# ucb-bar/Accelerated-TinyMPC

Measured on AMD Instinct MI355X. Metric: MPC solves/sec (batched quadrotor nx=12,nu=4,N=30), higher is better.
Workload: dtype f32; 1 GPU; quadrotor_tracking batched 65536 instances per GPU, cold-start tiny_solve, early_exit (tol 1e-3, max_iter 100); nx=12, nu=4, N=30, instances_per_gpu=65536, instances_total=65536, parallelism=batch-shard x1, world_size_seen=1, backend=none (single process), kernel=tile16<12,4,30,exact>, max_iters=85

## Files before the change

### accelerated-tinympc_amd/csrc/admm_tile16.hip

```cpp
#include "rowlane_math.h"
#include <cstdlib>

namespace tinympc
{

typedef float f32x16 __attribute__((ext_vector_type(16)));
#ifndef TINY_T16_ABLATE
#define TINY_T16_ABLATE 0
#endif
#ifndef TINY_T16_CQ
#define TINY_T16_CQ 1
#endif
#ifndef TINY_T16_BADDR
#define TINY_T16_BADDR 1
#endif
#ifndef TINY_T16_PADTAB
#define TINY_T16_PADTAB 1
#endif
#ifndef TINY_T16_XPOSE
#define TINY_T16_XPOSE 1
#endif
#ifndef TINY_T16_SCHED
#define TINY_T16_SCHED 1
#endif
#ifndef TINY_T16_LINES
#define TINY_T16_LINES 1
#endif
#ifndef TINY_T16_STAMP
#define TINY_T16_STAMP 0
#endif

#if TINY_T16_ABLATE == 1
__device__ __forceinline__ f32x4 t16_fake4(float a, float b, f32x4 c) { c[0] += a; c[1] += b; c[2] += a; c[3] += b; return c; }
#define TINY_MFMA4(a, b, c) t16_fake4((a), (b), (c))
#define TINY_MFMA1(a, b, c) __builtin_amdgcn_mfma_f32_16x16x1f32((a), (b), (c), 0, 0, 0)
#else
#define TINY_MFMA4(a, b, c) __builtin_amdgcn_mfma_f32_16x16x4f32((a), (b), (c), 0, 0, 0)
#define TINY_MFMA1(a, b, c) __builtin_amdgcn_mfma_f32_16x16x1f32((a), (b), (c), 0, 0, 0)
#endif

template <int V>
__device__ __forceinline__ void gather12(float (&t)[12], const f32x16 &p0, const f32x16 &p1, const f32x16 &p2)
{
#pragma unroll
    for (int b = 0; b < 4; b++)
    {
        t[b] = p0[4 * b + V];
        t[4 + b] = p1[4 * b + V];
        t[8 + b] = p2[4 * b + V];
    }
}
template <int V>
__device__ __forceinline__ void gather4(float (&t)[4], const f32x16 &p)
{
#pragma unroll
    for (int b = 0; b < 4; b++) t[b] = p[4 * b + V];
}

typedef float f32x2 __attribute__((ext_vector_type(2)));
// ... 235 lines not shown
                 : [m] "s"(m), [n0] "v"(pn[0]), [n1] "v"(pn[1]), [n2] "v"(pn[2]), [dd] "v"(dd)
                 : "scc");
}

__device__ __forceinline__ void masked_restore_slack(unsigned long long m, const float (&bo)[4], unsigned sn_addr)
{
    const f32x4 tv = {acc_get(bo[0]), acc_get(bo[1]), acc_get(bo[2]), acc_get(bo[3])};
    unsigned long long sx;
    asm volatile("s_and_saveexec_b64 %[sx], %[m]\n\t"
                 "ds_write_b128 %[ad], %[tv]\n\t"
                 "s_mov_b64 exec, %[sx]"
                 : [sx] "=&s"(sx)
                 : [m] "s"(m), [ad] "v"(sn_addr), [tv] "v"(tv)
                 : "memory", "scc");
}

template <bool EXACT>
__device__ __forceinline__ f32x4 lin_cost4(const f32x4 &cq, const f32x4 &rho4, const f32x4 &t1)
{
    if constexpr (EXACT) return cq - rho4 * t1;
    else return __builtin_elementwise_fma(-rho4, t1, cq);
}

__device__ __forceinline__ f32x4 t16_transpose4(const f32x4 &r)
{
    typedef unsigned u32x2 __attribute__((ext_vector_type(2)));
    const u32x2 a = __builtin_amdgcn_permlane32_swap(__float_as_uint(r[0]), __float_as_uint(r[2]), false, false);
    const u32x2 b = __builtin_amdgcn_permlane32_swap(__float_as_uint(r[1]), __float_as_uint(r[3]), false, false);
    const u32x2 lo = __builtin_amdgcn_permlane16_swap(a[0], b[0], false, false);
    const u32x2 hi = __builtin_amdgcn_permlane16_swap(a[1], b[1], false, false);
    return f32x4{__uint_as_float(lo[0]), __uint_as_float(lo[1]), __uint_as_float(hi[0]), __uint_as_float(hi[1])};
}

constexpr int TILE16_WAVES = 4;
constexpr int TILE16_MAX_TABLE_ROWS = 512;

__device__ __forceinline__ void t16_pair_lines(const f32x4 &e, const f32x4 &o, f32x4 &lo8, f32x4 &hi8)
{
#pragma unroll
    for (int k = 0; k < 4; k++)
    {
        lo8[k] = __int_as_float(__builtin_amdgcn_update_dpp(__float_as_int(e[k]), __float_as_int(o[k]), 0x128, 0xf, 0xc, false));
        hi8[k] = __int_as_float(__builtin_amdgcn_update_dpp(__float_as_int(o[k]), __float_as_int(e[k]), 0x128, 0xf, 0x3, false));
    }
}

#if TINY_T16_STAMP && !defined(TINY_T16_PI_UNIT)
constexpr int T16_STAMP_TILES = 32;
__device__ unsigned long long *t16_stamp_buf;
__device__ int t16_stamp_slots;
__device__ __forceinline__ void t16_stamp(int wslot, int k, int field, unsigned long long v)
{
    unsigned long long *const buf = t16_stamp_buf;
    if (buf && wslot < t16_stamp_slots && k < T16_STAMP_TILES && (threadIdx.x & 63) == 0) buf[((size_t)wslot * T16_STAMP_TILES + k) * 4 + field] = v;
}
#define T16_STAMP(k, field, v) t16_stamp((int)blockIdx.x * TILE16_WAVES + (int)(threadIdx.x >> 6), (k), (field), (v))
#else
#define T16_STAMP(k, field, v) ((void)0)
#endif

__device__ __forceinline__ void t16_dma_row(unsigned on, const float *sbase, unsigned voff, unsigned lds_dst, float after)
{
    asm volatile("s_cmp_eq_u32 %0, 0\n\ts_cbranch_scc1 1f\n\ts_mov_b32 m0, %3\n\ts_nop 0\n\tglobal_load_lds_dwordx4 %1, %2\n1:"
                 : : "s"(on), "v"(voff), "s"(sbase), "s"(lds_dst), "v"(after) : "memory", "scc");
}
__device__ __forceinline__ void t16_dma_row2(unsigned on, const float *sbase, unsigned voff, unsigned lds_dst, float after0, float after1)
{
    asm volatile("s_cmp_eq_u32 %0, 0\n\ts_cbranch_scc1 1f\n\ts_mov_b32 m0, %3\n\ts_nop 0\n\tglobal_load_lds_dwordx4 %1, %2\n\t"
                 "s_add_u32 m0, m0, 0x3f0\n\ts_nop 0\n\tglobal_load_lds_dwordx4 %1, %2 offset:16\n1:"
                 : : "s"(on), "v"(voff), "s"(sbase), "s"(lds_dst), "v"(after0), "v"(after1) : "memory", "scc");
}
__device__ __forceinline__ void t16_dma_img2(unsigned on, const float *sbase, unsigned voff, unsigned lds_dst, float after0, float after1)
{
    asm volatile("s_cmp_eq_u32 %0, 0\n\ts_cbranch_scc1 1f\n\ts_mov_b32 m0, %3\n\ts_nop 0\n\tglobal_load_lds_dwordx4 %1, %2\n\t"
                 "global_load_lds_dwordx4 %1, %2 offset:1024\n1:"
                 : : "s"(on), "v"(voff), "s"(sbase), "s"(lds_dst), "v"(after0), "v"(after1) : "memory", "scc");
}
__device__ __forceinline__ void t16_wait_vm(int k)
{
    if (k == 0) asm volatile("s_waitcnt vmcnt(0)" ::: "memory");
    else if (k == 1) asm volatile("s_waitcnt vmcnt(1)" ::: "memory");
    else if (k == 2) asm volatile("s_waitcnt vmcnt(2)" ::: "memory");
    else if (k == 3) asm volatile("s_waitcnt vmcnt(3)" ::: "memory");
    else if (k == 4) asm volatile("s_waitcnt vmcnt(4)" ::: "memory");
    else if (k == 5) asm volatile("s_waitcnt vmcnt(5)" ::: "memory");
    else if (k == 6) asm volatile("s_waitcnt vmcnt(6)" ::: "memory");
    else if (k == 7) asm volatile("s_waitcnt vmcnt(7)" ::: "memory");
// ... 233 lines not shown
            xr = load_xref(tabI, wsI, i);
        };
        auto make_lin = [&](int i, const float4 &sl, const f32x4 &xr) {
            const f32x4 sni = {sl.x, sl.y, sl.z, sl.w};
            return lin_cost4<EXACT>(cost_of(xr), rho4, sni - dual4(i));
        };
        float4 sl0; f32x4 xr0;
        load_lin(N - 2, sl0, xr0);
        f32x4 lin = make_lin(N - 2, sl0, xr0);
#pragma unroll
        for (int i = N - 2; i >= 0; i--)
        {
            float4 sl_n = make_float4(0.f, 0.f, 0.f, 0.f); f32x4 xr_n = {0.f, 0.f, 0.f, 0.f};
            if (EXACT && i > 0) load_lin(i - 1, sl_n, xr_n);
            typename TileMath<EXACT>::InFlight F;
            M.riccati_issue(p, lin, F);
            if (!EXACT && i > 0) load_lin(i - 1, sl_n, xr_n);
#if TINY_T16_SCHED
            if constexpr (EXACT) __builtin_amdgcn_sched_barrier(0);
#endif
            f32x4 lin_n = lin;
            if (i > 0) lin_n = make_lin(i - 1, sl_n, xr_n);
#if TINY_T16_SCHED
            if constexpr (EXACT) __builtin_amdgcn_sched_barrier(0);
#endif
            float pn[3], dd;
            M.riccati_finish(F, lin, pn, dd);
            masked_backward_update(amask, pl[i], dr[i], pn, dd);
            p[0] = pn[0]; p[1] = pn[1]; p[2] = pn[2];
            lin = lin_n;
        }
    };

    for (int ms = 0;; ++ms)
    {
    if (MPC && ms > 0) { st = TINY_STATUS_UNSOLVED_; itn = 1; }
    bool active = valid && (P.max_iter > 0);
    for (int it = 0; it < P.max_iter; ++it)
    {
        if (!__any(active)) break;
        int oz;
        asm volatile("s_mov_b32 %0, 0" : "=s"(oz));
        float4 *const snI = sn + oz;
        const float4 *bloI = blo + oz, *bhiI = bhi + oz;
        const float4 *const tabI = tab + oz;
        const int wsI = wstart + oz;
        const unsigned long long amask = __ballot(active);
        const unsigned sn_addr = (unsigned)(size_t)(lds_float4 *)snI;
        const unsigned gI = (sn_addr - (unsigned)__builtin_amdgcn_readfirstlane(sn_addr)) >> 8;
        const float4 *const bloG = bloI + gI, *const bhiG = bhiI + gI;
        const float *const bsrcI = P.bounds + oz, *const xsrcI = xsrc + oz;
        unsigned rdBI = 0, rdXI = 0;
        if constexpr (BR || XR)
        {
            const PiAddr AI = pi_addr(sn_addr - __builtin_amdgcn_readfirstlane(sn_addr));
            rdBI = COLD ? AI.rdB : A0.rdB + oz; rdXI = COLD ? AI.rdX : A0.rdX + oz;
        }
        const unsigned sB1 = onB ? T16_RING_B : 0u, sX1 = onX ? T16_RING_X : 0u;
        const unsigned sBlast = onB ? ((N - 1) % DB) * T16_RING_B : T16_RING_B;
        const unsigned lane16I = sn_addr - __builtin_amdgcn_readfirstlane(sn_addr);
        const unsigned timg = (unsigned)(tile_ok ? tile : 0) * (unsigned)N;
        unsigned xw = 0, bw = 0;
        if constexpr (XR) xw = timg * 1024u + (COLD ? lane16I : 16u * lane);
        if constexpr (BR) bw = timg * 2048u + (COLD ? lane16I : 16u * lane);
        auto dma_x = [&](int i, float after) { t16_dma_row(onX, xsrcI, xw + (unsigned)i * 1024u, dmaX + (i % DX) * T16_RING_X, after); };
        auto dma_b = [&](int i, float after0, float after1) { t16_dma_img2(onB, bsrcI, bw + (unsigned)i * 2048u, dmaB + (i % DB) * T16_RING_B, after0, after1); };
// ... 217 lines not shown
        continue;
    }

    {
        const bool solved = st == TINY_STATUS_SOLVED_;
        const int c2 = lane >> 2, q2 = lane & 3;
        const int inst2 = inst_of(c2);
        const bool valid2 = tile_ok && in_batch(inst2);
        const int obase2 = ((valid2 ? inst2 : 0) * N) * 16 + 4 * q2;
        typedef float float_ma __attribute__((may_alias));
        typedef f32x4 f32x4_ma __attribute__((may_alias));
        float_ma *const stage_w = reinterpret_cast<float_ma *>(lds4 + wv * (N * WAVE));
        const int rd_off = (c2 * 4 + q2);
        const int obase4 = ebase_e + 3 * g;
        constexpr bool XPOSE = TINY_T16_XPOSE && !(EXACT && !COLD && !MPC);
        auto put = [&](float *dst, int i, const f32x4 &val) {
            if constexpr (XPOSE)
            {
                const f32x4 o = t16_transpose4(val);
                if (valid_e) *reinterpret_cast<f32x4 *>(dst + obase4 + i * 16) = o;
                return;
            }
            float_ma *slot = stage_w + i * (WAVE * 4);
            reinterpret_cast<f32x4_ma *>(slot)[lane] = val;
            asm volatile("" ::: "memory");
            f32x4 o;
            o[0] = slot[rd_off]; o[1] = slot[rd_off + 64]; o[2] = slot[rd_off + 128]; o[3] = slot[rd_off + 192];
            asm volatile("" ::: "memory");
            if (valid2) *reinterpret_cast<f32x4 *>(dst + obase2 + i * 16) = o;
        };
        float s[3] = {x0[0], x0[1], x0[2]};
        if constexpr (XPOSE && TINY_T16_LINES && COLD && !MPC && !BR && !XR)
        {
            auto slack_of = [&](int i) { return reinterpret_cast<const f32x4_ma *>(stage_w + i * (WAVE * 4))[lane]; };
            auto lin_of = [&](int i, const f32x4 &sni) {
                const f32x4 xr = load_xref(tab, wstart, i);
                f32x4 lin = lin_cost4<EXACT>(cost_of(xr), rho4, sni - dual4(i));
                if (i == N - 1) lin[3] = 0.f;
                return lin;
            };
            auto pd_of = [&](int i) { return i == N - 1 ? f32x4{pN[0], pN[1], pN[2], 0.f} : f32x4{acc_get(pl[i][0]), acc_get(pl[i][1]), acc_get(pl[i][2]), dr[i]}; };
            auto vz_of = [&](int i, const f32x4 &sni) {
                f32x4 vzv;
    #pragma unroll
                for (int v = 0; v < 4; v++)
                {
                    const float bov = acc_get(bo[i][v]);
                    vzv[v] = solved ? bov : sni[v];
                }
                return vzv;
            };
            const int instL = inst_of(c & 7), instH = inst_of((c & 7) + 8);
            const bool validL = tile_ok && in_batch(instL), validH = tile_ok && in_batch(instH);
            const int obaseL = (validL ? instL : 0) * (N * 16) + ((c >> 3) << 4) + 4 * g;
            const int offH = ((validH ? instH : 0) - (validL ? instL : 0)) * (N * 16);
            auto put2 = [&](float *dst, int i, const f32x4 &ve, const f32x4 &vo) {
                f32x4 lo8, hi8;
                t16_pair_lines(t16_transpose4(ve), t16_transpose4(vo), lo8, hi8);
                if (validL) *reinterpret_cast<f32x4 *>(dst + obaseL + i * 16) = lo8;
                if (validH) *reinterpret_cast<f32x4 *>(dst + obaseL + offH + i * 16) = hi8;
            };
#pragma unroll
            for (int i = 0; i + 1 < N; i += 2)
            {
                const f32x4 sne = slack_of(i), sno = slack_of(i + 1);
                put2(P.gy, i, dual4(i), dual4(i + 1));
                put2(P.vzn, i, sne, sno);
                put2(P.vz, i, vz_of(i, sne), vz_of(i + 1, sno));
                put2(P.pd, i, pd_of(i), pd_of(i + 1));
                put2(P.qr, i, lin_of(i, sne), lin_of(i + 1, sno));
                float ue = 0.f, xe[3];
                M.lqr(s, dr[i], ue, xe);
                const f32x4 sve = {s[0], s[1], s[2], ue};
                float uo = 0.f, xo[3] = {0.f, 0.f, 0.f};
                if (i + 1 < N - 1) M.lqr(xe, dr[i + 1], uo, xo);
                put2(P.xu, i, sve, f32x4{xe[0], xe[1], xe[2], uo});
                s[0] = xo[0]; s[1] = xo[1]; s[2] = xo[2];
            }
            if constexpr (N % 2 == 1)
            {
                const f32x4 sni = slack_of(N - 1);
                put(P.xu, N - 1, f32x4{s[0], s[1], s[2], 0.f});
                put(P.qr, N - 1, lin_of(N - 1, sni));
                put(P.pd, N - 1, pd_of(N - 1));
                put(P.vz, N - 1, vz_of(N - 1, sni));
                put(P.vzn, N - 1, sni);
                put(P.gy, N - 1, dual4(N - 1));
            }
        }
        else
        {
#pragma unroll
        for (int i = 0; i < N; i++)
        {
            float un = 0.f, xn[3] = {0.f, 0.f, 0.f};
            if (i < N - 1) M.lqr(s, dr[i], un, xn);
            const f32x4 sv = {s[0], s[1], s[2], un};
            const f32x4 sni = reinterpret_cast<const f32x4_ma *>(stage_w + i * (WAVE * 4))[lane];
            const f32x4 xr = load_xref(tab, wstart, i);
            f32x4 lin = lin_cost4<EXACT>(cost_of(xr), rho4, sni - dual4(i));
            if (i == N - 1) lin[3] = 0.f;
            f32x4 pdv = {acc_get(pl[i][0]), acc_get(pl[i][1]), acc_get(pl[i][2]), dr[i]};
            if (i == N - 1) pdv = f32x4{pN[0], pN[1], pN[2], 0.f};
            f32x4 vzv;
#pragma unroll
            for (int v = 0; v < 4; v++)
            {
                const float bov = acc_get(bo[i][v]);
                vzv[v] = solved ? bov : sni[v];
            }
            put(P.xu, i, sv);
            put(P.qr, i, lin);
            put(P.pd, i, pdv);
            put(P.vz, i, vzv);
            put(P.vzn, i, sni);
            put(P.gy, i, dual4(i));
            if constexpr (!XPOSE) reinterpret_cast<f32x4_ma *>(stage_w + i * (WAVE * 4))[lane] = sni;
            s[0] = xn[0]; s[1] = xn[1]; s[2] = xn[2];
        }
        }
// ... 116 lines not shown
    return hipErrorInvalidValue;
}
#else
bool tile16_supported(int nx, int nu, int N)
{
    if (nx != 12 || nu != 4) return false;
#define TINY_TILE16_CHECK(NN) \
    if (N == NN) return true;
    TINY_FOR_EACH_TILE16(TINY_TILE16_CHECK)
    return false;
}

int tile16_max_table_rows() { return TILE16_MAX_TABLE_ROWS; }

bool tile16_two_ended(int batch, int n_cu, int tail)
{
    RowParams P{};
    static const int dummy_order = 0;
    P.batch = batch; P.cold_start = 1; P.mpc_steps = 1; P.order = &dummy_order;
    const int ntiles = (batch + 15) / 16;
    if (n_cu <= 0) n_cu = 256;
    const int want = (ntiles + TILE16_WAVES - 1) / TILE16_WAVES, nblocks = want < n_cu ? want : n_cu;
    return t16_tail_stride(P, ntiles, nblocks, tail, true) != 0u;
}

#if TINY_T16_STAMP
static int t16_stamp_nslots = 0;
extern "C" int tiny_t16_stamp_begin()
{
    static unsigned long long *buf = nullptr;
    int dev = 0, ncu = 0;
    if (hipGetDevice(&dev) != hipSuccess || hipDeviceGetAttribute(&ncu, hipDeviceAttributeMultiprocessorCount, dev) != hipSuccess || ncu <= 0) return 1;
    const int nslots = ncu * TILE16_WAVES;
    const size_t bytes = (size_t)nslots * T16_STAMP_TILES * 4 * sizeof(unsigned long long);
    if (buf) (void)hipFree(buf);
    buf = nullptr;
    if (hipMalloc(&buf, bytes) != hipSuccess || hipMemset(buf, 0, bytes) != hipSuccess) return 1;
    if (hipMemcpyToSymbol(HIP_SYMBOL(t16_stamp_slots), &nslots, sizeof(nslots)) != hipSuccess) return 1;
    if (hipMemcpyToSymbol(HIP_SYMBOL(t16_stamp_buf), &buf, sizeof(buf)) != hipSuccess || hipDeviceSynchronize() != hipSuccess) return 1;
    t16_stamp_nslots = nslots;
    return 0;
}
extern "C" int tiny_t16_stamp_slots() { return t16_stamp_nslots; }
extern "C" int tiny_t16_stamp_read(unsigned long long *host, int nslots)
{
    if (nslots > t16_stamp_nslots) return 1;
    unsigned long long *buf = nullptr;
    if (hipMemcpyFromSymbol(&buf, HIP_SYMBOL(t16_stamp_buf), sizeof(buf)) != hipSuccess || !buf) return 1;
    return hipMemcpy(host, buf, (size_t)nslots * T16_STAMP_TILES * 4 * sizeof(unsigned long long), hipMemcpyDeviceToHost) != hipSuccess;
}
extern "C" int tiny_t16_stamp_tiles() { return T16_STAMP_TILES; }
#endif

hipError_t launch_admm_tile16(int N, bool exact, const RowParams &P, hipStream_t stream, int n_cu, int tail)
{
    const int ntiles = (P.batch + 15) / 16;
    if (n_cu <= 0) n_cu = 256;
    const int want = (ntiles + TILE16_WAVES - 1) / TILE16_WAVES, nblocks = want < n_cu ? want : n_cu;
    const int rows = P.xref_mode == 1 ? P.table_rows : N;
    if (rows > TILE16_MAX_TABLE_ROWS) return hipErrorInvalidValue;
    const size_t lds = (size_t)(TILE16_WAVES * N * WAVE + 2 * N * 4 + (rows + N - 1) * 4) * sizeof(float4);
    RowParams Q = P;
    if (P.mpc_steps > 1 || !P.cold_start) Q.inst_map = nullptr;
    Q.pi_flags = (Q.pi_flags & 0xffu) | (t16_tail_stride(P, ntiles, nblocks, tail, Q.inst_map != nullptr) << 8);
#define TINY_TILE16_LAUNCH(NN, EX)                                                                                         \
    {                                                                                                                      \
        auto kern = P.mpc_steps > 1 ? (P.cold_start ? admm_tile16_kernel<NN, EX, true, true> : admm_tile16_kernel<NN, EX, false, true>) \
                                    : (P.cold_start ? admm_tile16_kernel<NN, EX, true> : admm_tile16_kernel<NN, EX, false>); \
        hipError_t e = hipFuncSetAttribute((const void *)kern, hipFuncAttributeMaxDynamicSharedMemorySize, (int)lds);      \
        if (e != hipSuccess) return e;                                                                                     \
        hipLaunchKernelGGL(kern, dim3(nblocks), dim3(WAVE * TILE16_WAVES), lds, stream, Q);                                \
        return hipGetLastError();                                                                                          \
    }
#define TINY_TILE16_DISPATCH(NN)                  \
    if (N == NN)                                  \
    {                                             \
        if (exact) TINY_TILE16_LAUNCH(NN, true)   \
        else TINY_TILE16_LAUNCH(NN, false)        \
    }
    TINY_FOR_EACH_TILE16(TINY_TILE16_DISPATCH)
    return hipErrorInvalidValue;
}
#endif

// ... 2 lines not shown
```

### accelerated-tinympc_amd/csrc/tinympc_batch.hip

```cpp
#include "../../include/tinympc_batch.h"
#include "eigen_orders.h"
#include "tinympc_internal.h"

#include <cmath>
#include <cstdarg>
#include <cstdio>
#include <cstring>
#include <limits>
#include <map>
#include <mutex>
#include <optional>
#include <string>
#include <vector>

using namespace tinympc;

namespace
{

thread_local std::string g_err;

int fail(int code, const char *fmt, ...)
{
    char buf[512];
// ... 388 lines not shown
    hipStream_t own_stream = nullptr;
    hipGraphExec_t graph_exec = nullptr;
    std::string graph_sig;
    bool have_cache = false, have_dyn = false, have_settings = false, gains_dirty = true;
    float rho = 0.f;
    std::vector<float> Kinf, Pinf, Quu_inv, AmBKt, Adyn, Bdyn, Q;
    float abs_pri_tol = 0.f, abs_dua_tol = 0.f;
    int max_iter = 0, check_termination = 1, en_state_bound = 0, en_input_bound = 0;
    int layout = LAYOUT_TILE;
    float *arr[TINY_ARR_COUNT] = {};
    float *pair[6] = {};
    size_t xfam_floats = 0, ufam_floats = 0, pair_floats = 0;
    InputArr in_xref, in_bnd[4];
    bool en_uref = false, en_d2p = false, have_rcost = false;
    std::vector<float> Rcost, coeff_d2p;
    InputArr in_uref;
    float *r_uref = nullptr;
    const int *order_dev = nullptr;
    int dispatch_mode = -1;
    float *u0_stage = nullptr;
    float *key_buf = nullptr;
    int *order_buf = nullptr;
    bool derived_dirty[2] = {true, true};
    float *t_xref = nullptr, *t_bnd[4] = {};
    float *r_xref = nullptr, *r_bounds = nullptr;
    float *r_bounds_img = nullptr, *r_xref_img = nullptr;
    size_t r_bounds_img_n = 0, r_xref_img_n = 0;
    int *rows_vary_dev = nullptr;
    unsigned rows_vary = 3u;
    size_t r_xref_n = 0, r_bounds_n = 0, r_uref_n = 0;
    int graph_captures = 0;
    int n_cu = 256;
    int tile_queue = -1;
    int tile_grouping = -1;
    int *tile_map = nullptr;
    bool tile_map_dirty = true;
    int tile_map_builds = 0;
    bool last_grouped = false;
    float *tab_tile = nullptr, *tab_row = nullptr;
    float *tab_row_h = nullptr;
    int table_rows = 0;
    int *xref_start = nullptr;
    int xref_mode = 0;
    float *res = nullptr;
    int *status = nullptr, *iter = nullptr, *n_unsolved = nullptr;
    float *opnd = nullptr, *qvec = nullptr;
    float *mats_exact = nullptr, *mats_fast = nullptr;
    float *dA = nullptr, *dB = nullptr;
    float *x0buf = nullptr;
    float *staging = nullptr;
    size_t staging_floats = 0;
    bool duals_zero_pending = false;
    bool cold_pending = false;
    bool x0_zero_pending = false;
    int variant = VAR_AUTO;
    std::optional<Kernel> row_family_forced;
    int last_dispatch = 0;
    bool iter_history = false;
    bool pm = false;
    float *pm_src = nullptr, *pm_rho = nullptr, *pm_row[2] = {};
    bool pm_row_dirty[2] = {true, true};
    bool h16 = false;
    bool dual32 = false;
    bool dual32_pref = false;
    bool dual32_forced = false;
    bool timing = false;
// ... 445 lines not shown
            if (!tb->rows_vary_dev) TRY(dev_alloc_zero((float **)&tb->rows_vary_dev, 2));
            HIP_TRY(hipMemsetAsync(tb->rows_vary_dev, 0, 2 * sizeof(int), tb->stream));
            hipLaunchKernelGGL(rows_vary_kernel, dim3(grid_for((long long)tb->batch * 16)), dim3(256), 0, tb->stream,
                               bounds_all_shared(tb) ? nullptr : reinterpret_cast<const float2 *>(tb->r_bounds), xper ? tb->r_xref : nullptr, tb->batch, N, nx, nu,
                               tb->rows_vary_dev);
            HIP_TRY(hipGetLastError());
            int h[2] = {1, 1};
            HIP_TRY(hipMemcpyAsync(h, tb->rows_vary_dev, sizeof h, hipMemcpyDeviceToHost, tb->stream));
            HIP_TRY(hipStreamSynchronize(tb->stream));
            tb->rows_vary = (h[0] ? 1u : 0u) | (h[1] ? 2u : 0u);
            const long long ntl = (tb->batch + 15) / 16;
            if (!bounds_all_shared(tb) && (tb->rows_vary & 1u))
            {
                TRY(sized_buffer(&tb->r_bounds_img, &tb->r_bounds_img_n, (size_t)ntl * N * 2 * 64 * 4));
                hipLaunchKernelGGL(tile16_image_kernel, dim3(grid_for(ntl * N * 128)), dim3(256), 0, tb->stream, reinterpret_cast<const float4 *>(tb->r_bounds),
                                   reinterpret_cast<float4 *>(tb->r_bounds_img), tb->batch, N, 2, (long long)N * 8);
                HIP_TRY(hipGetLastError());
            }
            if (xper && (tb->rows_vary & 2u))
            {
                TRY(sized_buffer(&tb->r_xref_img, &tb->r_xref_img_n, (size_t)ntl * N * 64 * 4));
                hipLaunchKernelGGL(tile16_image_kernel, dim3(grid_for(ntl * N * 64)), dim3(256), 0, tb->stream, reinterpret_cast<const float4 *>(tb->r_xref),
                                   reinterpret_cast<float4 *>(tb->r_xref_img), tb->batch, N, 1, (long long)N * 4);
                HIP_TRY(hipGetLastError());
            }
        }
    }
    HIP_TRY(hipStreamSynchronize(tb->stream));
    tb->derived_dirty[layout] = false;
    return 0;
}

constexpr int kTile16AutoPerCu = 160;
bool tile16_auto_size(const TinyBatch *tb) { return dispatch_effective(tb) == 1 && tb->batch >= kTile16AutoPerCu * tb->n_cu; }
constexpr int kTile16ClosedLoopPerCu = 160;
bool tile16_closed_loop_size(const TinyBatch *tb) { return tb->batch >= kTile16ClosedLoopPerCu * tb->n_cu; }

int settle_dual_width(TinyBatch *tb, bool kernel_keeps_fp32_duals)
{
    if (!tb->h16 || tb->dual32_forced) return 0;
    const bool want32 = tb->dual32_pref && kernel_keeps_fp32_duals;
    if (tb->dual32 == want32) return 0;
    if (tb->layout == LAYOUT_ROW && tb->pair[5])
    {
        float *nw = nullptr;
        TRY(dev_alloc_zero(&nw, want32 ? tb->pair_floats : (tb->pair_floats + 1) / 2));
        hipLaunchKernelGGL(dual_width_kernel, dim3(grid_for((long long)tb->pair_floats)), dim3(256), 0, tb->stream, tb->pair[5], nw, (long long)tb->pair_floats, want32 ? 1 : 0);
        HIP_TRY(hipGetLastError());
        HIP_TRY(hipStreamSynchronize(tb->stream));
        (void)guarded_free(tb->pair[5]);
        tb->pair[5] = nw;
    }
    tb->dual32 = want32;
    invalidate_graph(tb);
    return 0;
}

bool tile16_per_instance(const TinyBatch *tb)
{
    return !bounds_all_shared(tb) || (tb->xref_mode != 1 && tb->in_xref.set && !tb->in_xref.shared);
}
struct Tile16Pi { bool bounds_ring, xref_ring, fits; unsigned flags; };
Tile16Pi tile16_pi_plan(const TinyBatch *tb)
{
    Tile16Pi p;
    p.bounds_ring = !bounds_all_shared(tb);
// ... 338 lines not shown
    const bool predicted = eligible && want_predicted && !history && !pl.pm && !tb->dual32 && tb->max_iter > 1;
    if (traits(pl.kernel).order_unit_solve == 16) P.order = nullptr;
    P.inst_map = (!run && tb->tile_map && tile_grouping_wanted(tb, pl)) ? tb->tile_map : nullptr;
    hipError_t e = hipSuccess;
    if (history) e = launch_dispatch_order_history(tb->iter, tb->batch, unit, tb->order_buf, tb->n_unsolved, tb->stream, run && unit == 16);
    else if (predicted)
    {
        RowParams K;
        fill_row_params(tb, K, false);
        K.inst_map = P.inst_map;
        e = launch_dispatch_order(tb->nx, tb->nu, tb->h16, K, tb->key_buf, tb->order_buf, tb->stream, unit == 16);
    }
    else HIP_TRY(hipMemsetAsync(tb->n_unsolved, 0, 2 * sizeof(int), tb->stream));
    if (e != hipSuccess) return fail(TINY_BATCH_EHIP, "kernel launch failed: %s", hipGetErrorString(e));
    if (history || predicted) P.order = tb->order_buf;
    return history ? 3 : predicted ? 1 : (P.order ? 2 : 0);
}

hipError_t launch_kernel(const TinyBatch *tb, const KernelPlan &pl, RowParams &P)
{
    const int nx = tb->nx, nu = tb->nu, N = tb->N;
    switch (pl.kernel)
    {
    case Kernel::Rowlane:
        return pl.pm ? launch_admm_rowlane_pm(nx, nu, N, pl.exact, P, model_params(tb, pl), tb->stream) : launch_admm_rowlane(nx, nu, N, pl.exact, tb->h16, P, tb->stream);
    case Kernel::Rowloop: return launch_admm_rowloop(nx, nu, pl.exact, tb->h16, P, tb->stream);
    case Kernel::Rowstream: return launch_admm_rowstream(nx, nu, pl.exact, tb->h16, P, tb->stream);
    case Kernel::Wavestream: return launch_admm_wavestream(nx, nu, P, tb->stream);
    case Kernel::Quadlane: return launch_admm_quadlane(N, pl.exact, tb->h16, P, tb->stream);
    case Kernel::Waveres: return launch_admm_waveres(nx, nu, pl.exact, P, tb->stream);
    case Kernel::Tile48: return launch_admm_tile48(N, pl.exact, P, tb->stream);
    case Kernel::Tile16:
    {
        if (!pl.pi) return launch_admm_tile16(N, pl.exact, P, tb->stream, tb->n_cu, tb->tile_queue);
        const Tile16Pi &t = pl.pi_tables;
        P.pi_flags = t.flags;
        if (t.bounds_ring && (t.flags & 1u))
        {
            if (!tb->r_bounds_img) return hipErrorInvalidValue;
            P.bounds = tb->r_bounds_img;
        }
        if (t.xref_ring && (t.flags & 2u))
        {
            if (!tb->r_xref_img) return hipErrorInvalidValue;
            P.xref = tb->r_xref_img;
        }
        return launch_admm_tile16_pi(N, pl.exact, t.bounds_ring, t.xref_ring, P, tb->stream, tb->n_cu, tb->tile_queue);
    }
    case Kernel::Stream:
    case Kernel::Generic:
    {
        SolveParams S;
        fill_solve_params(tb, S);
        if (pl.kernel == Kernel::Stream) return launch_admm_stream(tb->NXC, tb->NUC, S, tb->stream);
        return pl.pm ? launch_admm_generic_pm(S, model_params(tb, pl), tb->NXC, tb->NUC, tb->stream) : launch_admm_generic(S, tb->gen_mats, tb->NXC, tb->NUC, tb->stream);
    }
    }
    return hipErrorInvalidValue;
}

int enqueue_solve(TinyBatch *tb, const KernelPlan &pl, bool record_events)
{
    const KernelTraits &t = traits(pl.kernel);
    RowParams P;
    if (t.layout == LAYOUT_ROW)
    {
        fill_row_params(tb, P, pl.exact);
        const int applied = enqueue_dispatch_order(tb, pl, 1, false, P);
        if (applied < 0) return applied;
        tb->last_dispatch = applied;
        tb->last_grouped = P.inst_map != nullptr;
    }
    else
    {
        HIP_TRY(hipMemsetAsync(tb->n_unsolved, 0, 2 * sizeof(int), tb->stream));
        tb->last_grouped = false;
    }
    if (record_events) HIP_TRY(hipEventRecord(tb->ev0, tb->stream));
    if (t.layout == LAYOUT_ROW && P.dual32 && !t.fp32_duals)
        return fail(TINY_BATCH_EUNSUPPORTED, "fp16 storage with fp32 duals runs on the register-resident 16-lane and quad kernels only "
// ... 906 lines not shown

int tiny_batch_debug_graph_captures(TinyBatch *tb)
{
    CHECK_TB(tb);
    return tb->graph_captures;
}

int tiny_batch_debug_guards(int on)
{
    std::lock_guard<std::mutex> lk(g_guard_mu);
    g_guards_on = on != 0;
    return 0;
}

long long tiny_batch_debug_check(void)
{
    std::lock_guard<std::mutex> lk(g_guard_mu);
    if (g_guarded.empty()) return 0;
    unsigned long long *bad = nullptr, host = 0;
    if (hipMalloc((void **)&bad, sizeof *bad) != hipSuccess || hipMemset(bad, 0, sizeof *bad) != hipSuccess) return fail(TINY_BATCH_EHIP, "tiny_batch_debug_check: allocation failed");
    if (hipDeviceSynchronize() != hipSuccess) { (void)hipFree(bad); return fail(TINY_BATCH_EHIP, "tiny_batch_debug_check: a kernel faulted: %s", hipGetErrorString(hipGetLastError())); }
    for (const auto &kv : g_guarded)
    {
        char *u = (char *)kv.first;
        hipLaunchKernelGGL(guard_count_kernel, dim3(1), dim3(256), 0, nullptr, (const unsigned *)(u - kGuard * sizeof(float)), kGuard, bad);
        hipLaunchKernelGGL(guard_count_kernel, dim3(1), dim3(256), 0, nullptr, (const unsigned *)(u + kv.second), kGuard, bad);
    }
    hipError_t e = hipMemcpy(&host, bad, sizeof host, hipMemcpyDeviceToHost);
    (void)hipFree(bad);
    if (e != hipSuccess) return fail(TINY_BATCH_EHIP, "tiny_batch_debug_check: %s", hipGetErrorString(e));
    return (long long)host;
}

int tiny_batch_debug_poke(TinyBatch *tb, int which)
{
    CHECK_TB(tb);
    TRY(set_device(tb));
    float *arr = tb->layout == LAYOUT_ROW ? tb->pair[0] : tb->arr[0];
    size_t bytes = 0;
    {
        std::lock_guard<std::mutex> lk(g_guard_mu);
        auto it = g_guarded.find(arr);
        if (it == g_guarded.end()) return fail(TINY_BATCH_ENOTREADY, "tiny_batch_debug_poke: the handle was not created under tiny_batch_debug_guards(1)");
        bytes = it->second;
    }
    const float v = 1.0f;
    HIP_TRY(hipMemcpy(which ? (char *)arr + bytes : (char *)arr - sizeof(float), &v, sizeof v, hipMemcpyHostToDevice));
    return 0;
}

int tiny_batch_arithmetic(TinyBatch *tb)
{
    CHECK_TB(tb);
    KernelPlan pl;
    TRY(resolve_plan(tb, false, &pl));
    return pl.exact ? TINY_BATCH_ARITH_EXACT : TINY_BATCH_ARITH_FMA;
}

const char *tiny_batch_closed_loop_kernel_name(TinyBatch *tb)
{
    if (!tb) return "";
    return plan_name(tb, true);
}

int tiny_batch_set_row_kernel(TinyBatch *tb, int family)
{
// ... 73 lines not shown
```

### accelerated-tinympc_amd/solver.py

```python
from __future__ import annotations

import ctypes as C
from pathlib import Path

import numpy as np

import os

from . import build as _build

PKG = Path(__file__).resolve().parent
LIB_PATH = PKG / "lib" / "libtinympc_hip.so"

ARRAY_IDS = {"x": 0, "u": 1, "q": 2, "r": 3, "p": 4, "d": 5, "v": 6, "vnew": 7, "z": 8, "znew": 9, "g": 10, "y": 11}
X_FAMILY = ("x", "q", "p", "v", "vnew", "g")
TINY_SOLVED, TINY_UNSOLVED = 1, 11

_lib = None


class TinyBatchError(RuntimeError):
    pass


# ... 8 lines not shown
            raise TinyBatchError(f"{LIB_PATH} is missing: run `python accelerated-tinympc_amd/build.py` "
                                 "(hipcc --offload-arch=gfx950); there is no CPU fallback")
    override = os.environ.get("TINYMPC_HIP_LIB")
    if override:
        import warnings
        warnings.warn(f"TINYMPC_HIP_LIB is set: loading {override} instead of {LIB_PATH}", RuntimeWarning)
    lib = C.CDLL(override or str(LIB_PATH))
    F, I, P = C.POINTER(C.c_float), C.POINTER(C.c_int), C.c_void_p
    D = C.POINTER(C.c_double)
    sig = {
        "tiny_batch_create": [C.POINTER(P), C.c_int, C.c_int, C.c_int, C.c_int, C.c_int],
        "tiny_batch_set_stream": [P, P],
        "tiny_batch_synchronize": [P],
        "tiny_batch_set_cache": [P, C.c_float, F, F, F, F],
        "tiny_batch_set_dynamics": [P, F, F, F],
        "tiny_batch_set_settings": [P, C.c_float, C.c_float, C.c_int, C.c_int, C.c_int, C.c_int],
        "tiny_batch_set_x0": [P, F],
        "tiny_batch_set_xref": [P, F, C.c_int],
        "tiny_batch_set_xref_window": [P, F, C.c_int, I],
        "tiny_batch_set_umin": [P, F, C.c_int], "tiny_batch_set_umax": [P, F, C.c_int],
        "tiny_batch_set_xmin": [P, F, C.c_int], "tiny_batch_set_xmax": [P, F, C.c_int],
        "tiny_batch_reset_dual_variables": [P],
        "tiny_batch_solve": [P], "tiny_batch_solve_async": [P], "tiny_batch_wait": [P, I],
        "tiny_batch_get_x": [P, F], "tiny_batch_get_u": [P, F],
        "tiny_batch_forward_pass": [P], "tiny_batch_update_slack": [P], "tiny_batch_update_dual": [P],
        "tiny_batch_update_linear_cost": [P], "tiny_batch_backward_pass_grad": [P], "tiny_batch_termination_condition": [P, I],
        "tiny_batch_get_status": [P, I, I, F], "tiny_batch_set_status": [P, I, I, F],
        "tiny_batch_set_array": [P, C.c_int, F], "tiny_batch_get_array": [P, C.c_int, F],
        "tiny_batch_reset_workspace": [P],
        "tiny_batch_set_x0_device": [P, P], "tiny_batch_get_u0_device": [P, P],
        "tiny_batch_mpc_step_async": [P, C.c_int], "tiny_batch_get_x0": [P, F],
        "tiny_batch_mpc_run_async": [P, C.c_int, C.c_int], "tiny_batch_mpc_run_traj_async": [P, C.c_int, C.c_int, P], "tiny_batch_mpc_run_traj": [P, C.c_int, C.c_int, F],
        "tiny_batch_enable_timing": [P, C.c_int], "tiny_batch_last_solve_ms": [P, F],
        "tiny_batch_select_kernel": [P, C.c_int], "tiny_batch_arithmetic": [P], "tiny_batch_debug_graph_captures": [P], "tiny_batch_set_storage": [P, C.c_int], "tiny_batch_set_storage_ex": [P, C.c_int, C.c_int],
        "tiny_batch_set_row_kernel": [P, C.c_int],
        "tiny_batch_set_dispatch": [P, C.c_int], "tiny_batch_set_tile_queue": [P, C.c_int], "tiny_batch_set_tile_grouping": [P, C.c_int], "tiny_batch_tile_grouping_applied": [P], "tiny_batch_get_tile_map": [P, I, I], "tiny_batch_set_dispatch_order_device": [P, P], "tiny_batch_dispatch_applied": [P],
        "tiny_batch_set_optional_terms": [P, C.c_int, C.c_int], "tiny_batch_set_input_cost": [P, F],
        "tiny_batch_set_coeff_d2p": [P, F], "tiny_batch_set_uref": [P, F, C.c_int],
        "tiny_batch_group_solve": [C.POINTER(P), C.c_int, I],
        "tiny_batch_group_gather_u0": [C.POINTER(P), C.c_int, C.c_int, P], "tiny_batch_group_get_u0": [C.POINTER(P), C.c_int, F],
        "tiny_batch_set_array_device": [P, C.c_int, P], "tiny_batch_get_array_device": [P, C.c_int, P],
        "tiny_batch_set_xref_device": [P, P, C.c_int],
        "tiny_riccati": [C.c_int, C.c_int, D, D, D, D, C.c_double, D, D, D, D, D, I],
        "tiny_batch_set_models": [P, F, F, F, F, F, F, F, F], "tiny_batch_set_models_device": [P, P, P, P, P, P, P, P, P],
        "tiny_batch_clear_models": [P], "tiny_batch_models_per_instance": [P],
        "tiny_batch_riccati_device": [C.c_int, C.c_int, C.c_int, P, P, P, P, P, P, P, P, P, P, P, P],
        "tiny_batch_set_systems": [P, D, D, D, D, D, I],
    }
    for name, args in sig.items():
        fn = getattr(lib, name)
        fn.argtypes, fn.restype = args, C.c_int
    sig64 = {
        "tiny_batch64_create": [C.POINTER(P), C.c_int, C.c_int, C.c_int, C.c_int, C.c_int],
        "tiny_batch64_set_cache": [P, C.c_double, D, D, D, D], "tiny_batch64_set_dynamics": [P, D, D, D],
        "tiny_batch64_set_settings": [P, C.c_double, C.c_double, C.c_int, C.c_int, C.c_int, C.c_int],
        "tiny_batch64_set_x0": [P, D], "tiny_batch64_set_xref": [P, D, C.c_int],
        "tiny_batch64_set_xmin": [P, D, C.c_int], "tiny_batch64_set_xmax": [P, D, C.c_int],
        "tiny_batch64_set_umin": [P, D, C.c_int], "tiny_batch64_set_umax": [P, D, C.c_int],
        "tiny_batch64_reset_dual_variables": [P], "tiny_batch64_solve": [P],
        "tiny_batch64_set_array": [P, C.c_int, D], "tiny_batch64_get_array": [P, C.c_int, D],
        "tiny_batch64_get_status": [P, I, I, D], "tiny_batch64_set_status": [P, I, I, D],
        "tiny_batch64_select_kernel": [P, C.c_int], "tiny_batch64_mpc_step": [P], "tiny_batch64_get_first_columns": [P, D, D],
        "tiny_batch64_forward_pass": [P], "tiny_batch64_update_slack": [P], "tiny_batch64_update_dual": [P],
        "tiny_batch64_update_linear_cost": [P], "tiny_batch64_backward_pass_grad": [P], "tiny_batch64_termination_condition": [P, I],
        "tiny_batch64_set_xref_window": [P, D, C.c_int, I], "tiny_batch64_get_xref_start": [P, I],
        "tiny_batch64_mpc_run": [P, C.c_int, C.c_int], "tiny_batch64_mpc_run_traj": [P, C.c_int, C.c_int, D],
    }
# ... 321 lines not shown

    def enable_timing(self, on=True):
        self._check(self.lib.tiny_batch_enable_timing(self._h, 1 if on else 0))

    def last_solve_ms(self) -> float:
        ms = C.c_float(0)
        self._check(self.lib.tiny_batch_last_solve_ms(self._h, C.byref(ms)))
        return ms.value

    def kernel_name(self) -> str:
        return self.lib.tiny_batch_kernel_name(self._h).decode()

    def closed_loop_kernel_name(self) -> str:
        return self.lib.tiny_batch_closed_loop_kernel_name(self._h).decode()

    def arithmetic(self) -> str:
        rc = self.lib.tiny_batch_arithmetic(self._h)
        if rc < 0:
            self._check(rc)
        return "exact" if rc == 0 else "fma"

    def select_kernel(self, variant: int):
        self._check(self.lib.tiny_batch_select_kernel(self._h, variant))

    def set_row_kernel(self, family: int):
        self._check(self.lib.tiny_batch_set_row_kernel(self._h, family))

    def set_dispatch(self, mode: int):
        self._check(self.lib.tiny_batch_set_dispatch(self._h, mode))

    def set_tile_queue(self, stride: int):
        self._check(self.lib.tiny_batch_set_tile_queue(self._h, stride))

    def set_tile_grouping(self, mode: int):
        self._check(self.lib.tiny_batch_set_tile_grouping(self._h, mode))

    def tile_grouping_applied(self) -> bool:
        return bool(self._check(self.lib.tiny_batch_tile_grouping_applied(self._h)))

    def tile_map(self):
        builds = C.c_int(0)
        n = self._check(self.lib.tiny_batch_get_tile_map(self._h, None, C.byref(builds)))
        if n == 0:
            return None, builds.value
        m = np.empty(n, np.int32)
        self._check(self.lib.tiny_batch_get_tile_map(self._h, m.ctypes.data_as(C.POINTER(C.c_int)), None))
        return m, builds.value

    def dispatch_applied(self) -> int:
        return self._check(self.lib.tiny_batch_dispatch_applied(self._h))

    def set_dispatch_order_device(self, d_order_ptr):
        self._check(self.lib.tiny_batch_set_dispatch_order_device(self._h, C.c_void_p(d_order_ptr)))

    def set_storage(self, bits: int, dual_bits: int | None = None):
        if dual_bits is None:
            self._check(self.lib.tiny_batch_set_storage(self._h, bits))
        else:
            self._check(self.lib.tiny_batch_set_storage_ex(self._h, bits, dual_bits))

    def set_stream(self, stream_ptr: int):
        self._check(self.lib.tiny_batch_set_stream(self._h, C.c_void_p(stream_ptr)))


class TinyBatchSolver64:

# ... 140 lines not shown
```

### include/tinympc_batch.h

```cpp
#ifndef TINYMPC_BATCH_H
#define TINYMPC_BATCH_H

#ifdef __cplusplus
extern "C"
{
#endif

    typedef struct TinyBatch TinyBatch;

    typedef enum
    {
        TINY_BATCH_OK = 0,
        TINY_BATCH_EINVAL = -1,
        TINY_BATCH_EHIP = -2,
        TINY_BATCH_EUNSUPPORTED = -3,
        TINY_BATCH_ENOTREADY = -4
    } TinyBatchError;

#define TINY_STATUS_SOLVED 1
#define TINY_STATUS_UNSOLVED 11

    typedef enum
    {
        TINY_ARR_X = 0, TINY_ARR_U = 1, TINY_ARR_Q = 2, TINY_ARR_R = 3, TINY_ARR_P = 4, TINY_ARR_D = 5,
// ... 38 lines not shown

    int tiny_batch_solve_async(TinyBatch *tb);
    int tiny_batch_wait(TinyBatch *tb, int *n_unsolved);

    int tiny_batch_group_solve(TinyBatch **tbs, int n, int *n_unsolved);
    int tiny_batch_group_gather_u0(TinyBatch **tbs, int n, int dst_device, float *d_dst);
    int tiny_batch_group_get_u0(TinyBatch **tbs, int n, float *u0_host);

    int tiny_batch_set_array(TinyBatch *tb, int array_id, const float *src);
    int tiny_batch_get_array(TinyBatch *tb, int array_id, float *dst);
    int tiny_batch_set_status(TinyBatch *tb, const int *iter, const int *status, const float *residuals);
    int tiny_batch_reset_workspace(TinyBatch *tb);

    int tiny_batch_set_x0_device(TinyBatch *tb, const float *d_x0 );
    int tiny_batch_get_u0_device(TinyBatch *tb, float *d_u0 );
    int tiny_batch_set_array_device(TinyBatch *tb, int array_id, const float *d_src);
    int tiny_batch_get_array_device(TinyBatch *tb, int array_id, float *d_dst);
    int tiny_batch_set_xref_device(TinyBatch *tb, const float *d_xref , int shared);

    int tiny_batch_mpc_step_async(TinyBatch *tb, int window_advance);
    int tiny_batch_mpc_run_async(TinyBatch *tb, int steps, int window_advance);
    int tiny_batch_mpc_run_traj_async(TinyBatch *tb, int steps, int window_advance, float *d_u0_traj);
    int tiny_batch_mpc_run_traj(TinyBatch *tb, int steps, int window_advance, float *u0_traj_host);
    int tiny_batch_get_x0(TinyBatch *tb, float *x0 );

    int tiny_batch_enable_timing(TinyBatch *tb, int on);
    int tiny_batch_last_solve_ms(TinyBatch *tb, float *ms);
    const char *tiny_batch_kernel_name(TinyBatch *tb);
    const char *tiny_batch_closed_loop_kernel_name(TinyBatch *tb);
    int tiny_batch_debug_guards(int on);
    int tiny_batch_debug_graph_captures(TinyBatch *tb);
    long long tiny_batch_debug_check(void);
    int tiny_batch_debug_poke(TinyBatch *tb, int which);
    enum { TINY_BATCH_ARITH_EXACT = 0, TINY_BATCH_ARITH_FMA = 1 };
    int tiny_batch_arithmetic(TinyBatch *tb);
    int tiny_batch_select_kernel(TinyBatch *tb, int variant);
    int tiny_batch_set_row_kernel(TinyBatch *tb, int family);
    int tiny_batch_set_storage(TinyBatch *tb, int bits);
    int tiny_batch_set_storage_ex(TinyBatch *tb, int bits, int dual_bits);

    int tiny_batch_set_dispatch(TinyBatch *tb, int mode);
    int tiny_batch_set_tile_queue(TinyBatch *tb, int stride);
    int tiny_batch_set_tile_grouping(TinyBatch *tb, int mode);
    int tiny_batch_tile_grouping_applied(TinyBatch *tb);
    int tiny_batch_get_tile_map(TinyBatch *tb, int *map, int *builds);
    int tiny_batch_dispatch_applied(TinyBatch *tb);
    int tiny_batch_set_dispatch_order_device(TinyBatch *tb, const int *d_order);

    int tiny_batch_set_optional_terms(TinyBatch *tb, int en_uref, int en_coeff_d2p);
    int tiny_batch_set_input_cost(TinyBatch *tb, const float *R);
    int tiny_batch_set_coeff_d2p(TinyBatch *tb, const float *coeff_d2p);
    int tiny_batch_set_uref(TinyBatch *tb, const float *uref, int shared);

    int tiny_batch_set_models(TinyBatch *tb, const float *rho , const float *Kinf , const float *Pinf ,
                              const float *Quu_inv , const float *AmBKt , const float *Adyn ,
                              const float *Bdyn , const float *Q );
    int tiny_batch_set_models_device(TinyBatch *tb, const float *d_rho, const float *d_Kinf, const float *d_Pinf, const float *d_Quu_inv,
                                     const float *d_AmBKt, const float *d_Adyn, const float *d_Bdyn, const float *d_Q);
    int tiny_batch_clear_models(TinyBatch *tb);
    int tiny_batch_models_per_instance(TinyBatch *tb);
    int tiny_batch_riccati_device(int nx, int nu, int count, const double *d_A, const double *d_B, const double *d_Q, const double *d_R,
                                  const double *d_rho, double *d_Kinf, double *d_Pinf, double *d_Quu_inv, double *d_AmBKt,
                                  double *d_coeff_d2p, int *d_iters, void *hip_stream);
    int tiny_batch_set_systems(TinyBatch *tb, const double *A, const double *B, const double *Q, const double *R, const double *rho, int *iters);

    int tiny_riccati(int nx, int nu, const double *A, const double *B, const double *Q, const double *R, double rho,
// ... 7 lines not shown
```

Measured before the change: 47.95 million solves/s.

## Pipeline final output writeback through LDS staging for full tiles

Adds a full-tile path for the cold-start output epilogue. Each pair of rows is staged into per-wave LDS, then read back transposed and written as 16-byte global stores, with the staging of the next output array interleaved ahead of the fetch and store of the previous one. Values are forced into fresh registers and the lane index is made opaque so the compiler does not stretch live ranges across the epilogue. The goal is to overlap output-store latency with computation and lower register pressure, at the cost of extra LDS traffic. The change also adds stamp fields and a debug workgroup cap, neither of which is used by default.

```diff
diff --git a/accelerated-tinympc_amd/csrc/admm_tile16.hip b/accelerated-tinympc_amd/csrc/admm_tile16.hip
--- a/accelerated-tinympc_amd/csrc/admm_tile16.hip
+++ b/accelerated-tinympc_amd/csrc/admm_tile16.hip
@@ -25,6 +25,9 @@
 #endif
 #ifndef TINY_T16_LINES
 #define TINY_T16_LINES 1
+#endif
+#ifndef TINY_T16_LIVEOUT
+#define TINY_T16_LIVEOUT 1
 #endif
 #ifndef TINY_T16_STAMP
 #define TINY_T16_STAMP 0
@@ -326,6 +329,13 @@
     return f32x4{__uint_as_float(lo[0]), __uint_as_float(lo[1]), __uint_as_float(hi[0]), __uint_as_float(hi[1])};
 }
 
+__device__ __forceinline__ float t16_fresh(float v)
+{
+    float r;
+    asm("v_mov_b32 %0, %1" : "=v"(r) : "v"(v));
+    return r;
+}
+
 constexpr int TILE16_WAVES = 4;
 constexpr int TILE16_MAX_TABLE_ROWS = 512;
 
@@ -341,12 +351,13 @@
 
 #if TINY_T16_STAMP && !defined(TINY_T16_PI_UNIT)
 constexpr int T16_STAMP_TILES = 32;
+constexpr int T16_STAMP_FIELDS = 6;
 __device__ unsigned long long *t16_stamp_buf;
 __device__ int t16_stamp_slots;
 __device__ __forceinline__ void t16_stamp(int wslot, int k, int field, unsigned long long v)
 {
     unsigned long long *const buf = t16_stamp_buf;
-    if (buf && wslot < t16_stamp_slots && k < T16_STAMP_TILES && (threadIdx.x & 63) == 0) buf[((size_t)wslot * T16_STAMP_TILES + k) * 4 + field] = v;
+    if (buf && wslot < t16_stamp_slots && k < T16_STAMP_TILES && (threadIdx.x & 63) == 0) buf[((size_t)wslot * T16_STAMP_TILES + k) * T16_STAMP_FIELDS + field] = v;
 }
 #define T16_STAMP(k, field, v) t16_stamp((int)blockIdx.x * TILE16_WAVES + (int)(threadIdx.x >> 6), (k), (field), (v))
 #else
@@ -646,6 +657,7 @@
         }
     };
 
+    T16_STAMP(stamp_k, 4, __builtin_amdgcn_s_memrealtime());
     for (int ms = 0;; ++ms)
     {
     if (MPC && ms > 0) { st = TINY_STATUS_UNSOLVED_; itn = 1; }
@@ -929,9 +941,17 @@
         float s[3] = {x0[0], x0[1], x0[2]};
         if constexpr (XPOSE && TINY_T16_LINES && COLD && !MPC && !BR && !XR)
         {
+#if TINY_T16_LIVEOUT
+            unsigned lq = lane;
+            asm volatile("" : "+v"(lq));
+            const int lane = (int)lq, g = (int)(lq >> 4), c = (int)(lq & 15u);
+            const int gx = g;
+#else
+            const int gx = -1;
+#endif
             auto slack_of = [&](int i) { return reinterpret_cast<const f32x4_ma *>(stage_w + i * (WAVE * 4))[lane]; };
             auto lin_of = [&](int i, const f32x4 &sni) {
-                const f32x4 xr = load_xref(tab, wstart, i);
+                const f32x4 xr = load_xref(tab, wstart, i, gx);
                 f32x4 lin = lin_cost4<EXACT>(cost_of(xr), rho4, sni - dual4(i));
                 if (i == N - 1) lin[3] = 0.f;
                 return lin;
@@ -957,6 +977,95 @@
                 if (validL) *reinterpret_cast<f32x4 *>(dst + obaseL + i * 16) = lo8;
                 if (validH) *reinterpret_cast<f32x4 *>(dst + obaseL + offH + i * 16) = hi8;
             };
+#if TINY_T16_LIVEOUT
+            const bool full_tile = __all(validL && validH) != 0 && P.batch <= (int)(0xffffffffu / (N * 64u));
+            if (full_tile)
+            {
+                unsigned lf = lane;
+                asm volatile("" : "+v"(lf));
+                f32x4_ma *const wr0 = reinterpret_cast<f32x4_ma *>(stage_w) + lf;
+                const float_ma *const rd0 = stage_w + (((lf >> 3) & 1u) << 8) + ((lf & 7u) << 2) + (lf >> 4);
+                auto stage = [&](int ar, const f32x4 &ve, const f32x4 &vo) { wr0[ar * WAVE] = ve; wr0[(ar + 1) * WAVE] = vo; };
+                auto fetch = [&](int ar, f32x4 &lo8, f32x4 &hi8) {
+                    const float_ma *rp = rd0 + ar * (WAVE * 4);
+                    asm volatile("" ::: "memory");
+#pragma unroll
+                    for (int r = 0; r < 4; r++) { lo8[r] = rp[64 * r]; hi8[r] = rp[64 * r + 32]; }
+                    asm volatile("" ::: "memory");
+                };
+                const unsigned boL = (unsigned)obaseL * 4u, boH = (unsigned)(obaseL + offH) * 4u;
+                auto emit = [&](float *dst, int i, const f32x4 &lo8, const f32x4 &hi8) {
+                    *reinterpret_cast<f32x4 *>(reinterpret_cast<char *>(dst) + (size_t)boL + i * 64) = lo8;
+                    *reinterpret_cast<f32x4 *>(reinterpret_cast<char *>(dst) + (size_t)boH + i * 64) = hi8;
+                };
+#pragma unroll
+                for (int i = 0; i + 1 < N; i += 2)
+                {
+                    const bool piped = i >= 2;
+                    const int arA = i, arB = piped ? i - 2 : i;
+                    const f32x4 sne = slack_of(i), sno = slack_of(i + 1);
+                    auto round = [&](float *dst, int ar, auto &&stage_next) {
+                        if (piped) stage_next();
+                        f32x4 lo8, hi8;
+                        fetch(ar, lo8, hi8);
+                        emit(dst, i, lo8, hi8);
+                        if (!piped) stage_next();
+                    };
+                    auto fresh4 = [&](const f32x4 &q) { return f32x4{t16_fresh(q[0]), t16_fresh(q[1]), t16_fresh(q[2]), t16_fresh(q[3])}; };
+                    stage(arA, fresh4(dual4(i)), fresh4(dual4(i + 1)));
+                    round(P.gy, arA, [&] { stage(arB, sne, sno); });
+                    round(P.vzn, arB, [&] {
+                        const f32x4 vze = vz_of(i, sne), vzo = vz_of(i + 1, sno);
+#pragma unroll
+                        for (int v = 0; v < 4; v++) { acc_put(bo[i][v], sne[v]); acc_put(bo[i + 1][v], sno[v]); }
+                        stage(arA, vze, vzo);
+                    });
+                    round(P.vz, arA, [&] {
+                        f32x4 pde = pd_of(i), pdo = pd_of(i + 1);
+                        if (i < N - 1) pde[3] = t16_fresh(pde[3]);
+                        if (i + 1 < N - 1) pdo[3] = t16_fresh(pdo[3]);
+                        stage(arB, pde, pdo);
+                    });
+                    round(P.pd, arB, [&] { stage(arA, lin_of(i, sne), lin_of(i + 1, sno)); });
+                    round(P.qr, arA, [&] {
+                        float ue = 0.f, xe[3];
+                        M.lqr(s, dr[i], ue, xe);
+                        const f32x4 sve = {s[0], s[1], s[2], ue};
+                        float uo = 0.f, xo[3] = {0.f, 0.f, 0.f};
+                        if (i + 1 < N - 1) M.lqr(xe, dr[i + 1], uo, xo);
+                        stage(arB, sve, f32x4{xe[0], xe[1], xe[2], uo});
+                        s[0] = xo[0]; s[1] = xo[1]; s[2] = xo[2];
+                    });
+                    if (i + 3 >= N) T16_STAMP(stamp_k, 5, __builtin_amdgcn_s_memrealtime());
+                    round(P.xu, arB, [&] {});
+#if TINY_T16_SCHED
+                    __builtin_amdgcn_sched_barrier(0);
+#endif
+                }
+                if constexpr (N % 2 == 1)
+                {
+                    auto put1 = [&](float *dst, const f32x4 &val) { *reinterpret_cast<f32x4 *>(dst + obase4 + (N - 1) * 16) = t16_transpose4(val); };
+                    const f32x4 sni = slack_of(N - 1);
+                    put1(P.xu, f32x4{s[0], s[1], s[2], 0.f});
+                    put1(P.qr, lin_of(N - 1, sni));
+                    put1(P.pd, pd_of(N - 1));
+                    put1(P.vz, vz_of(N - 1, sni));
+                    put1(P.vzn, sni);
+                    put1(P.gy, dual4(N - 1));
+                }
+                if (__ballot(valid_e && !solved) != 0ull)
+                {
+#pragma unroll
+                    for (int i = 0; i + 1 < N; i += 2)
+                    {
+                        wr0[i * WAVE] = f32x4{acc_get(bo[i][0]), acc_get(bo[i][1]), acc_get(bo[i][2]), acc_get(bo[i][3])};
+                        wr0[(i + 1) * WAVE] = f32x4{acc_get(bo[i + 1][0]), acc_get(bo[i + 1][1]), acc_get(bo[i + 1][2]), acc_get(bo[i + 1][3])};
+                    }
+                }
+            }
+            else
+#endif
+            {
 #pragma unroll
             for (int i = 0; i + 1 < N; i += 2)
             {
@@ -971,6 +1080,7 @@
                 const f32x4 sve = {s[0], s[1], s[2], ue};
                 float uo = 0.f, xo[3] = {0.f, 0.f, 0.f};
                 if (i + 1 < N - 1) M.lqr(xe, dr[i + 1], uo, xo);
+                if (i + 3 >= N) T16_STAMP(stamp_k, 5, __builtin_amdgcn_s_memrealtime());
                 put2(P.xu, i, sve, f32x4{xe[0], xe[1], xe[2], uo});
                 s[0] = xo[0]; s[1] = xo[1]; s[2] = xo[2];
             }
@@ -983,6 +1093,7 @@
                 put(P.vz, N - 1, vz_of(N - 1, sni));
                 put(P.vzn, N - 1, sni);
                 put(P.gy, N - 1, dual4(N - 1));
+            }
             }
         }
         else
@@ -1165,7 +1276,7 @@
     int dev = 0, ncu = 0;
     if (hipGetDevice(&dev) != hipSuccess || hipDeviceGetAttribute(&ncu, hipDeviceAttributeMultiprocessorCount, dev) != hipSuccess || ncu <= 0) return 1;
     const int nslots = ncu * TILE16_WAVES;
-    const size_t bytes = (size_t)nslots * T16_STAMP_TILES * 4 * sizeof(unsigned long long);
+    const size_t bytes = (size_t)nslots * T16_STAMP_TILES * T16_STAMP_FIELDS * sizeof(unsigned long long);
     if (buf) (void)hipFree(buf);
     buf = nullptr;
     if (hipMalloc(&buf, bytes) != hipSuccess || hipMemset(buf, 0, bytes) != hipSuccess) return 1;
@@ -1180,9 +1291,10 @@
     if (nslots > t16_stamp_nslots) return 1;
     unsigned long long *buf = nullptr;
     if (hipMemcpyFromSymbol(&buf, HIP_SYMBOL(t16_stamp_buf), sizeof(buf)) != hipSuccess || !buf) return 1;
-    return hipMemcpy(host, buf, (size_t)nslots * T16_STAMP_TILES * 4 * sizeof(unsigned long long), hipMemcpyDeviceToHost) != hipSuccess;
+    return hipMemcpy(host, buf, (size_t)nslots * T16_STAMP_TILES * T16_STAMP_FIELDS * sizeof(unsigned long long), hipMemcpyDeviceToHost) != hipSuccess;
 }
 extern "C" int tiny_t16_stamp_tiles() { return T16_STAMP_TILES; }
+extern "C" int tiny_t16_stamp_fields() { return T16_STAMP_FIELDS; }
 #endif
 
 hipError_t launch_admm_tile16(int N, bool exact, const RowParams &P, hipStream_t stream, int n_cu, int tail)
diff --git a/accelerated-tinympc_amd/csrc/tinympc_batch.hip b/accelerated-tinympc_amd/csrc/tinympc_batch.hip
--- a/accelerated-tinympc_amd/csrc/tinympc_batch.hip
+++ b/accelerated-tinympc_amd/csrc/tinympc_batch.hip
@@ -444,6 +444,7 @@
     int graph_captures = 0;
     int n_cu = 256;
     int tile_queue = -1;
+    int debug_workgroups = 0;
     int tile_grouping = -1;
     int *tile_map = nullptr;
     bool tile_map_dirty = true;
@@ -955,6 +956,7 @@
 }
 
 constexpr int kTile16AutoPerCu = 160;
+static int tile16_workgroups(const TinyBatch *tb) { return tb->debug_workgroups > 0 && tb->debug_workgroups < tb->n_cu ? tb->debug_workgroups : tb->n_cu; }
 bool tile16_auto_size(const TinyBatch *tb) { return dispatch_effective(tb) == 1 && tb->batch >= kTile16AutoPerCu * tb->n_cu; }
 constexpr int kTile16ClosedLoopPerCu = 160;
 bool tile16_closed_loop_size(const TinyBatch *tb) { return tb->batch >= kTile16ClosedLoopPerCu * tb->n_cu; }
@@ -1359,7 +1361,7 @@
     case Kernel::Tile48: return launch_admm_tile48(N, pl.exact, P, tb->stream);
     case Kernel::Tile16:
     {
-        if (!pl.pi) return launch_admm_tile16(N, pl.exact, P, tb->stream, tb->n_cu, tb->tile_queue);
+        if (!pl.pi) return launch_admm_tile16(N, pl.exact, P, tb->stream, tile16_workgroups(tb), tb->tile_queue);
         const Tile16Pi &t = pl.pi_tables;
         P.pi_flags = t.flags;
         if (t.bounds_ring && (t.flags & 1u))
@@ -1372,7 +1374,7 @@
             if (!tb->r_xref_img) return hipErrorInvalidValue;
             P.xref = tb->r_xref_img;
         }
-        return launch_admm_tile16_pi(N, pl.exact, t.bounds_ring, t.xref_ring, P, tb->stream, tb->n_cu, tb->tile_queue);
+        return launch_admm_tile16_pi(N, pl.exact, t.bounds_ring, t.xref_ring, P, tb->stream, tile16_workgroups(tb), tb->tile_queue);
     }
     case Kernel::Stream:
     case Kernel::Generic:
@@ -2345,6 +2347,15 @@
     return (long long)host;
 }
 
+int tiny_batch_debug_set_workgroups(TinyBatch *tb, int n)
+{
+    CHECK_TB(tb);
+    if (n < 0) return fail(TINY_BATCH_EINVAL, "tiny_batch_debug_set_workgroups: n must be 0 (one workgroup per compute unit) or a positive cap");
+    tb->debug_workgroups = n;
+    invalidate_graph(tb);
+    return TINY_BATCH_OK;
+}
+
 int tiny_batch_debug_poke(TinyBatch *tb, int which)
 {
     CHECK_TB(tb);
diff --git a/accelerated-tinympc_amd/solver.py b/accelerated-tinympc_amd/solver.py
--- a/accelerated-tinympc_amd/solver.py
+++ b/accelerated-tinympc_amd/solver.py
@@ -64,7 +64,7 @@
         "tiny_batch_mpc_step_async": [P, C.c_int], "tiny_batch_get_x0": [P, F],
         "tiny_batch_mpc_run_async": [P, C.c_int, C.c_int], "tiny_batch_mpc_run_traj_async": [P, C.c_int, C.c_int, P], "tiny_batch_mpc_run_traj": [P, C.c_int, C.c_int, F],
         "tiny_batch_enable_timing": [P, C.c_int], "tiny_batch_last_solve_ms": [P, F],
-        "tiny_batch_select_kernel": [P, C.c_int], "tiny_batch_arithmetic": [P], "tiny_batch_debug_graph_captures": [P], "tiny_batch_set_storage": [P, C.c_int], "tiny_batch_set_storage_ex": [P, C.c_int, C.c_int],
+        "tiny_batch_select_kernel": [P, C.c_int], "tiny_batch_arithmetic": [P], "tiny_batch_debug_graph_captures": [P], "tiny_batch_debug_set_workgroups": [P, C.c_int], "tiny_batch_set_storage": [P, C.c_int], "tiny_batch_set_storage_ex": [P, C.c_int, C.c_int],
         "tiny_batch_set_row_kernel": [P, C.c_int],
         "tiny_batch_set_dispatch": [P, C.c_int], "tiny_batch_set_tile_queue": [P, C.c_int], "tiny_batch_set_tile_grouping": [P, C.c_int], "tiny_batch_tile_grouping_applied": [P], "tiny_batch_get_tile_map": [P, I, I], "tiny_batch_set_dispatch_order_device": [P, P], "tiny_batch_dispatch_applied": [P],
         "tiny_batch_set_optional_terms": [P, C.c_int, C.c_int], "tiny_batch_set_input_cost": [P, F],
@@ -452,6 +452,9 @@
     def set_tile_queue(self, stride: int):
         self._check(self.lib.tiny_batch_set_tile_queue(self._h, stride))
 
+    def debug_set_workgroups(self, n: int):
+        self._check(self.lib.tiny_batch_debug_set_workgroups(self._h, n))
+
     def set_tile_grouping(self, mode: int):
         self._check(self.lib.tiny_batch_set_tile_grouping(self._h, mode))
 
diff --git a/include/tinympc_batch.h b/include/tinympc_batch.h
--- a/include/tinympc_batch.h
+++ b/include/tinympc_batch.h
@@ -94,6 +94,7 @@
     int tiny_batch_debug_graph_captures(TinyBatch *tb);
     long long tiny_batch_debug_check(void);
     int tiny_batch_debug_poke(TinyBatch *tb, int which);
+    int tiny_batch_debug_set_workgroups(TinyBatch *tb, int n);
     enum { TINY_BATCH_ARITH_EXACT = 0, TINY_BATCH_ARITH_FMA = 1 };
     int tiny_batch_arithmetic(TinyBatch *tb);
     int tiny_batch_select_kernel(TinyBatch *tb, int variant);
```

New measurement: 48.08 million solves/s (median of 6 runs). Within noise of the previous version (+0.3%).
